# kfjahnke/envutil

Hardware: AMD Instinct MI355X
Metric: Mpix/s reprojected (16K lat/lon->cubemap, b-spline-3) (higher is better)
Workload: dtype f32

## Files before the change

### envutil_amd/csrc/eu_render4.hip

```cpp
#include <cstdio>
#include <cstring>
#include <vector>
#include <algorithm>
#include "eu_packed_dev.h"
#include "eu_launch.h"

#define EU4_TW 16
#define EU4_TH 8
#define EU4_WAVES 4
#ifndef EU4_WAVES0
#define EU4_WAVES0 1
#define EU4_TEXELS 384
#define EU4_OCC0 4
#endif
#define EU4_UNIT_ROWS 4
#define EU4_COL_FLOATS 8
#define EU4_MAX_PLANS 16

__device__ __forceinline__ void eu4_box_reduce(int &mn0, int &mn1, int &mx0, int &mx1)
{
#define EU4_RED(ctrl)                                        \
  "v_min_i32_dpp %0, %0, %0 " ctrl "\n\t"                    \
  "v_min_i32_dpp %1, %1, %1 " ctrl "\n\t"                    \
  "v_max_i32_dpp %2, %2, %2 " ctrl "\n\t"                    \
  "v_max_i32_dpp %3, %3, %3 " ctrl "\n\t"
  asm("s_nop 1\n\t"
      EU4_RED("row_shr:1 row_mask:0xf bank_mask:0xf")
      EU4_RED("row_shr:2 row_mask:0xf bank_mask:0xf")
      EU4_RED("row_shr:4 row_mask:0xf bank_mask:0xf")
      EU4_RED("row_shr:8 row_mask:0xf bank_mask:0xf")
      EU4_RED("row_bcast:15 row_mask:0xa bank_mask:0xf")
      EU4_RED("row_bcast:31 row_mask:0xc bank_mask:0xf")
      "s_nop 0"
      : "+v"(mn0), "+v"(mn1), "+v"(mx0), "+v"(mx1));
#undef EU4_RED
  mn0 = __builtin_amdgcn_readlane(mn0, 63); mn1 = __builtin_amdgcn_readlane(mn1, 63);
  mx0 = __builtin_amdgcn_readlane(mx0, 63); mx1 = __builtin_amdgcn_readlane(mx1, 63);
}

typedef __attribute__((address_space(3))) void *eu4_lds_void;
typedef const __attribute__((address_space(1))) void *eu4_gbl_void;

typedef float eu4_f4 __attribute__((ext_vector_type(4)));

__device__ __forceinline__ void eu4_dma_row(unsigned dst, unsigned voff, const char *sb)
{
  unsigned keep;
  asm volatile("s_mov_b32 %0, m0\n\t"
               "s_mov_b32 m0, %1\n\t"
               "s_nop 0\n\t"
               "global_load_lds_dwordx4 %2, %3\n\t"
               "s_mov_b32 m0, %0"
               : "=&s"(keep) : "s"(dst), "v"(voff), "s"(sb) : "memory");
}

struct eu4_plan {
  const float *atab_g;
  const int *tileplan;
  const float *coltab;
  int tiles16;
  const int *l2_rows;
  int l2_off[9];
  int l2_half;
  unsigned long long l2_magic;
  const int *l1_ent;
  int l1_off[9];
  int l1_ecols;
  unsigned long long l1_magic;
  const int *xtab;
  const int *boxtab;
#ifdef EU5_STAMPS
  unsigned long long *stamps;
#endif
};

#ifdef EU5_STAMPS
#define EU5_STAMP(k) do { asm volatile("" ::: "memory"); st_[k] = __builtin_amdgcn_s_memtime(); asm volatile("" ::: "memory"); } while (0)
#define EU5_STAMP32(k) do { asm volatile("" ::: "memory"); st_[k] = (unsigned)__builtin_amdgcn_s_memtime(); asm volatile("" ::: "memory"); } while (0)
#else
#define EU5_STAMP(k) do { } while (0)
#define EU5_STAMP32(k) do { } while (0)
#endif

template <int NCH, int DEG, int PRJ>
__device__ __forceinline__ void eu4_tile(const eu_render_params &p, const eu4_plan &w, const float *atab,
                                         float *wtile, int tile_y, int x0, int lane)
{
  constexpr int TEX = 4;
  constexpr int order = DEG + 1;
  const eu_src_dev &s = p.src;
  const int lx = lane & 7, ly = lane >> 3;
  const int y = p.row_begin + tile_y * EU4_TH + ly;
  const bool yin = y < p.row_end;
  const int yc = yin ? y : p.row_end - 1;
  const float *rt = p.row + (long long)eu_frame_row(yc, p.band_shift, p.band_count, p.band_index) * EU_ROW_FLOATS;
  const int xa = x0 + 2 * lx, xb = xa + 1;
  const bool va = yin && xa < p.width, vb = yin && xb < p.width;
  const int xac = xa < p.width ? xa : p.width - 1, xbc = xb < p.width ? xb : p.width - 1;

  eu_f2 tx, ty, gy;
  eu_i2 hit, ok = { -1, -1 };
  int ixa, ixb;
  float wxa[order], wxb[order];
  eu_ray2 r;
  {
    const float A0 = rt[0], A1 = rt[1], A2 = rt[2], B0 = rt[3], B1 = rt[4], B2 = rt[5];
    const eu_f2 c0 = { p.col[xac], p.col[xbc] };
    if (p.form == EU_FORM_BCA) {
      const float C0 = rt[6], C1 = rt[7], C2 = rt[8];
      const float *colB = p.col + p.width;
      const eu_f2 c1 = { colB[xac], colB[xbc] };
      r.x = B0 * c0 + C0 * c1 + A0;
      r.y = B1 * c0 + C1 * c1 + A1;
      r.z = B2 * c0 + C2 * c1 + A2;
    } else {
      r.x = B0 * c0 + A0;
      r.y = B1 * c0 + A1;
// ... 114 lines not shown
  if constexpr (EU4_WAVES0 > 1) {
    asm volatile("s_waitcnt vmcnt(0)" ::: "memory");
    __syncthreads();
  }
  if (tile_x >= w.tiles16) return;
  eu4_tile<NCH, DEG, PRJ>(p, w, atab, tile, tile_y, tile_x * EU4_TW, lane);
}

template <int NCH, int DEG, int PRJ>
__device__ __forceinline__ void eu4_direct_tile(const eu_render_params &p, const float *atab, int tile_y, int x0, int lane)
{
  const eu_src_dev &s = p.src;
  const int lx = lane & 7, ly = lane >> 3;
  const int y = p.row_begin + tile_y * EU4_TH + ly;
  const bool yin = y < p.row_end;
  const int yc = yin ? y : p.row_end - 1;
  const float *rt = p.row + (long long)eu_frame_row(yc, p.band_shift, p.band_count, p.band_index) * EU_ROW_FLOATS;
  const int xa = x0 + 2 * lx, xb = xa + 1;
  const bool va = yin && xa < p.width, vb = yin && xb < p.width;
  const int xac = xa < p.width ? xa : p.width - 1, xbc = xb < p.width ? xb : p.width - 1;
  eu_ray2 ry;
  {
    const float A0 = rt[0], A1 = rt[1], A2 = rt[2], B0 = rt[3], B1 = rt[4], B2 = rt[5];
    const eu_f2 c0 = { p.col[xac], p.col[xbc] };
    if (p.form == EU_FORM_BCA) {
      const float C0 = rt[6], C1 = rt[7], C2 = rt[8];
      const float *colB = p.col + p.width;
      const eu_f2 c1 = { colB[xac], colB[xbc] };
      ry.x = B0 * c0 + C0 * c1 + A0;
      ry.y = B1 * c0 + C1 * c1 + A1;
      ry.z = B2 * c0 + C2 * c1 + A2;
    } else {
      ry.x = B0 * c0 + A0;
      ry.y = B1 * c0 + A1;
      ry.z = B2 * c0 + A2;
    }
    if (p.norm_mode == EU_NORM_DIV) {
      eu_f2 sqn = ry.x * ry.x; sqn = sqn + ry.y * ry.y; sqn = sqn + ry.z * ry.z;
      const eu_f2 n = { sqrtf(sqn.x), sqrtf(sqn.y) };
      ry.x = ry.x / n; ry.y = ry.y / n; ry.z = ry.z / n;
    }
  }
  eu_f2 sx, sy;
  eu_i2 hit = eu_coord2<PRJ>(s, ry, sx, sy, atab);
  hit = hit & (eu_i2){ va ? -1 : 0, vb ? -1 : 0 };
  float pxa[NCH], pxb[NCH];
  eu_eval2<NCH, DEG>(s, sx, sy, hit, pxa, pxb);
  float *const orow = p.out + (long long)(yc - p.row_begin) * p.out_stride;
  if (va) eu_put<NCH>(orow, xa, pxa);
  if (vb) eu_put<NCH>(orow, xb, pxb);
}

#include "eu_share_groups.h"
#include "eu_render5.h"

template <int DEG>
__global__ __launch_bounds__(256) void eu_colplan_kernel(const eu_render_params p, float *ct,
                                                         float A0, float A2, float B0, float B2)
{
  __shared__ __attribute__((aligned(16))) float atab[EU_ATAN_TAB_FLOATS];
  if (threadIdx.x < EU_ATAN_TAB_ENTRIES) eu_atan_tab_entry(threadIdx.x, atab + 8 * threadIdx.x);
  __syncthreads();
  constexpr int order = DEG + 1;
  const eu_src_dev &s = p.src;
  const int xa = 2 * (blockIdx.x * 256 + threadIdx.x), xb = xa + 1;
  if (xa >= p.width) return;
  const int xbc = xb < p.width ? xb : p.width - 1;
  const eu_f2 c0 = { p.col[xa], p.col[xbc] };
  const eu_f2 rx = B0 * c0 + A0, rz = B2 * c0 + A2;
  eu_i2 ok = { -1, -1 };
  const eu_f2 q2 = rx * rx + rz * rz;
  const eu_f2 qs = eu_sqrt2_ok(q2, ok);
  const eu_f2 lon = eu_atan2f_2_tab_ok(rx, rz, atab, 0, ok);
  eu_f2 i0 = { (float)((double)lon.x - s.tex_x0), (float)((double)lon.y - s.tex_x0) };
  if (s.cdiv_ok) i0 = eu_div2_const(i0, s.ext_w, s.rcp_ext_w);
  else i0 = i0 / s.ext_w;
  i0 = i0 * s.total_w; i0 = i0 - .5f;
  const eu_f2 sx = i0 - s.win_x_off;
  const eu_f2 gx = eu_gate2_ok(sx, s.gate0, s.lower0, s.upper0, ok);
  eu_f2 fx;
  if constexpr (DEG & 1) fx = (eu_f2){ floorf(gx.x), floorf(gx.y) };
  else fx = (eu_f2){ roundf(gx.x), roundf(gx.y) };
  const eu_f2 tx = gx - fx;
  eu_f2 wx[4];
#pragma unroll
  for (int i = 0; i < 4; i++) wx[i] = (eu_f2){ 0.0f, 0.0f };
  if constexpr (DEG >= 2) eu_weights2<DEG>(s.wm, tx, wx);
  float e[2][EU4_COL_FLOATS];
  e[0][0] = __int_as_float(ok.x ? (int)fx.x : INT_MIN);
  e[1][0] = __int_as_float(ok.y ? (int)fx.y : INT_MIN);
  e[0][1] = tx.x; e[1][1] = tx.y;
#pragma unroll
  for (int i = 0; i < 4; i++) { e[0][2 + i] = i < order ? wx[i].x : 0.0f; e[1][2 + i] = i < order ? wx[i].y : 0.0f; }
  e[0][6] = qs.x; e[1][6] = qs.y;
  e[0][7] = lon.x; e[1][7] = lon.y;
  float *o = ct + (size_t)xa * EU4_COL_FLOATS;
#pragma unroll
  for (int i = 0; i < EU4_COL_FLOATS; i++) o[i] = e[0][i];
  if (xb < p.width) {
#pragma unroll
    for (int i = 0; i < EU4_COL_FLOATS; i++) o[EU4_COL_FLOATS + i] = e[1][i];
  }
}

template <int NCH, int DEG, int PRJ>
__global__ __launch_bounds__(256, 4) void eu_render4d_kernel(const eu_render_params p, const eu4_plan w)
// ... 63 lines not shown
      static const int occ = [] { int n = 0; return hipOccupancyMaxActiveBlocksPerMultiprocessor(&n, eu_render5_kernel<NCH, DEG, PRJ, true>, 64 * EU5_WAVES, 0) == hipSuccess ? n : 0; }();
      per_cu = occ;
    } else {
      static const int occ = [] { int n = 0; return hipOccupancyMaxActiveBlocksPerMultiprocessor(&n, eu_render5_kernel<NCH, DEG, PRJ, false>, 64 * EU5_WAVES, 0) == hipSuccess ? n : 0; }();
      per_cu = occ;
    }
    const int wgs = (cus / 8) * 8 * per_cu;
    if (wgs <= 0) return -1;
    if (fast) eu4_followers_last = eu4_followers_plan;
    eu4_boxtab_last = bt;
    if (bt) hipLaunchKernelGGL((eu_render5_kernel<NCH, DEG, PRJ, true, true>), dim3((unsigned)wgs), dim3(64 * EU5_WAVES), 0, st, p, w);
    else if (fast) hipLaunchKernelGGL((eu_render5_kernel<NCH, DEG, PRJ, true>), dim3((unsigned)wgs), dim3(64 * EU5_WAVES), 0, st, p, w);
    else hipLaunchKernelGGL((eu_render5_kernel<NCH, DEG, PRJ, false>), dim3((unsigned)wgs), dim3(64 * EU5_WAVES), 0, st, p, w);
  } else {
    const int units = (p.tiles_y + EU4_UNIT_ROWS - 1) / EU4_UNIT_ROWS;
    dim3 grid((unsigned)(8 * ((w.tiles16 + EU4_WAVES0 - 1) / EU4_WAVES0)), (unsigned)EU4_UNIT_ROWS, (unsigned)((units + 7) / 8));
    hipLaunchKernelGGL((eu_render4s_kernel<NCH, DEG, PRJ>), grid, dim3(64 * EU4_WAVES0), 0, st, p, w);
  }
  if (hipGetLastError() != hipSuccess) return -1;
  hipLaunchKernelGGL((eu_render4d_kernel<NCH, DEG, PRJ>), dim3(EU4_DIRECT_WGS), dim3(256), 0, st, p, w);
  if (hipGetLastError() != hipSuccess) {
    (void)hipMemsetAsync(p.wl, 0, EU4_WL_ENTRIES * sizeof(int), st);
    return -1;
  }
  return 0;
}

template <int NCH, int DEG>
static int launch4_nd(const eu_render_params &p, const eu4_plan &w, hipStream_t st)
{
  switch (p.src.prj) {
    case EU_SPHERICAL: return launch4_ndp<NCH, DEG, EU_SPHERICAL>(p, w, st);
    case EU_CUBEMAP: return launch4_ndp<NCH, DEG, EU_CUBEMAP>(p, w, st);
    case EU_BIATAN6: return launch4_ndp<NCH, DEG, EU_BIATAN6>(p, w, st);
  }
  return -2;
}

template <int NCH>
static int launch4_n(const eu_render_params &p, const eu4_plan &w, hipStream_t st)
{
  switch (p.src.degree) {
    case 1: return launch4_nd<NCH, 1>(p, w, st);
    case 2: return launch4_nd<NCH, 2>(p, w, st);
    case 3: return launch4_nd<NCH, 3>(p, w, st);
  }
  return -2;
}

static_assert(EU_STAGED_TILE_ROWS == EU4_TH && EU_STAGED_MAX_TILES_Y == 65535 * 8 * EU4_UNIT_ROWS, "eu_select.h: eu_staged_covers");
namespace {
struct plan_cache {
  std::vector<unsigned char> key;
  eu_dev_buf<int> tileplan, l2_rows, l1_ent, xtab, boxtab;
  bool has_boxtab = false;
  long long boxtab_tiles = 0;
  eu_dev_buf<float> coltab;
  float *atab = nullptr;
  int planned_rows = 0;
  int l2_off[9] = {};
  int l1_off[9] = {};
  int l1_ecols = 1;
  long long follower_tiles = 0;
  hipStream_t last_stream = nullptr;
} g4s[EU_MAX_SLOTS];
#define g4 (g4s[eu_current_slot()])

bool ensure_atab()
{
  if (g4.atab) return true;
  std::vector<float> tab(768, 0.0f);
  for (int i = 0; i < EU_ATAN_TAB_ENTRIES; i++) eu_atan_tab_entry(i, tab.data() + 8 * i);
  if (hipMalloc((void **)&g4.atab, tab.size() * sizeof(float)) != hipSuccess) return false;
  return hipMemcpy(g4.atab, tab.data(), tab.size() * sizeof(float), hipMemcpyHostToDevice) == hipSuccess;
}

template <int DEG>
void launch_colplan(const eu_render_params &p, float *ct, const float *k, hipStream_t st)
{
  hipLaunchKernelGGL((eu_colplan_kernel<DEG>), dim3((unsigned)((p.width + 511) / 512)), dim3(256), 0, st, p, ct,
                     k[0], k[1], k[2], k[3]);
}

std::vector<unsigned char> eu4_plan_key(const eu_render_params &p, unsigned long long plan_gen, const eu_switches &sw)
{
  std::vector<unsigned char> key(sizeof(unsigned long long) + sizeof(eu_src_dev) + 11 * sizeof(int));
  unsigned char *q = key.data();
  memcpy(q, &plan_gen, sizeof plan_gen); q += sizeof plan_gen;
  eu_src_dev sd = p.src; sd.base = nullptr;
  memcpy(q, &sd, sizeof sd); q += sizeof sd;
  const int v[11] = { p.width, p.row_begin, p.row_end, p.band_shift, p.band_count, p.band_index, p.form, p.norm_mode, sw.share,
                      sw.boxtab, sw.boxtab_max_kb };
  memcpy(q, v, sizeof v);
  return key;
}

bool upload(eu_dev_buf<int> &buf, const std::vector<int> &v, size_t spare)
{
  if (buf.reserve(v.size() + spare) != hipSuccess) return false;
  return v.empty() || hipMemcpy(buf.p, v.data(), v.size() * sizeof(int), hipMemcpyHostToDevice) == hipSuccess;
}

template <int DEG>
void launch_boxplan(const eu_render_params &p, const float *atab_g, const int *l2_rows, int tiles16, int ntiles, int *tab, hipStream_t st)
{
  hipLaunchKernelGGL((eu5_boxplan_kernel<DEG>), dim3((unsigned)((ntiles + 3) / 4)), dim3(256), 0, st, p, atab_g, l2_rows, tiles16,
                     ntiles, tab);
}

int eu4_build_plans(const eu_render_params &p, int tiles16, const eu_switches &sw, const float *h_row,
                    size_t h_row_floats, hipStream_t st)
{
  std::vector<int> tp((size_t)p.tiles_y, -1);
  std::vector<float> plans;
  const bool can = p.form == EU_FORM_BA && p.norm_mode == EU_NORM_NONE && h_row;
  if (can && sw.colplan) {
    for (int ty = 0; ty < p.tiles_y; ty++) {
      float k[4] = { 0, 0, 0, 0 };
      bool same = true;
      for (int ly = 0; ly < EU4_TH && same; ly++) {
        const int y = std::min(p.row_begin + ty * EU4_TH + ly, p.row_end - 1);
        const size_t fr = (size_t)eu_frame_row(y, p.band_shift, p.band_count, p.band_index) * EU_ROW_FLOATS;
        if (fr + 6 > h_row_floats) { same = false; break; }
        const float c[4] = { h_row[fr + 0], h_row[fr + 2], h_row[fr + 3], h_row[fr + 5] };
        if (ly == 0) memcpy(k, c, sizeof k);
        else same = memcmp(k, c, sizeof k) == 0;
      }
      if (!same) continue;
      int id = -1;
      for (size_t j = 0; j < plans.size() / 4 && id < 0; j++)
        if (memcmp(&plans[4 * j], k, sizeof k) == 0) id = (int)j;
      if (id < 0 && plans.size() / 4 < EU4_MAX_PLANS) {
        id = (int)(plans.size() / 4);
        plans.insert(plans.end(), k, k + 4);
      }
      tp[(size_t)ty] = id;
    }
  }
  const int nplans = (int)(plans.size() / 4);
  if (g4.tileplan.reserve(tp.size()) != hipSuccess) return -1;
  if (g4.coltab.reserve(std::max<size_t>(1, nplans) * (size_t)p.width * EU4_COL_FLOATS) != hipSuccess) return -1;
  if (hipStreamSynchronize(st) != hipSuccess) return -1;
  if (g4.last_stream && g4.last_stream != st && hipStreamSynchronize(g4.last_stream) != hipSuccess) return -1;
  if (hipMemcpy(g4.tileplan.p, tp.data(), tp.size() * sizeof(int), hipMemcpyHostToDevice) != hipSuccess) return -1;
  g4.planned_rows = 0;
  for (int v : tp) g4.planned_rows += v >= 0;
  auto paired = [&](int m) { return 2 * m + 1 < p.tiles_y && tp[(size_t)2 * m] >= 0 && tp[(size_t)2 * m] == tp[(size_t)2 * m + 1]; };
  {
    std::vector<int> rows[8], all;
    for (int r = 0; r < p.tiles_y; r++)
      if (!paired(r >> 1)) rows[(r / EU5_UNIT_ROWS) & 7].push_back(r);
    for (int x = 0; x < 8; x++) { g4.l2_off[x] = (int)all.size(); all.insert(all.end(), rows[x].begin(), rows[x].end()); }
    g4.l2_off[8] = (int)all.size();
    if (!upload(g4.l2_rows, all, 1)) return -1;
  }
  g4.has_boxtab = false; g4.boxtab_tiles = 0;
  if (sw.boxtab && eu_staged_fast_profile(p)) {
    const long long ntiles = (long long)g4.l2_off[8] * tiles16;
    const long long bytes = ntiles * (EU5_BT_RECS * 16);
    if (bytes <= (long long)sw.boxtab_max_kb * 1024) {
      if (g4.boxtab.reserve((size_t)std::max<long long>(1, ntiles) * (EU5_BT_RECS * 4)) != hipSuccess) return -1;
      if (ntiles > 0) {
        switch (p.src.degree) {
          case 1: launch_boxplan<1>(p, g4.atab, g4.l2_rows.p, tiles16, (int)ntiles, g4.boxtab.p, st); break;
          case 2: launch_boxplan<2>(p, g4.atab, g4.l2_rows.p, tiles16, (int)ntiles, g4.boxtab.p, st); break;
          default: launch_boxplan<3>(p, g4.atab, g4.l2_rows.p, tiles16, (int)ntiles, g4.boxtab.p, st); break;
        }
        if (hipGetLastError() != hipSuccess) return -1;
      }
      g4.has_boxtab = true; g4.boxtab_tiles = ntiles;
    }
  }
  for (int j = 0; j < nplans; j++) {
    float *ct = g4.coltab.p + j * (size_t)p.width * EU4_COL_FLOATS;
    switch (p.src.degree) {
      case 1: launch_colplan<1>(p, ct, &plans[4 * j], st); break;
      case 2: launch_colplan<2>(p, ct, &plans[4 * j], st); break;
      default: launch_colplan<3>(p, ct, &plans[4 * j], st); break;
    }
    if (hipGetLastError() != hipSuccess) return -1;
  }
  std::vector<float> h_ct((size_t)nplans * p.width * EU4_COL_FLOATS);
  if (nplans) {
    if (hipStreamSynchronize(st) != hipSuccess) return -1;
    if (hipMemcpy(h_ct.data(), g4.coltab.p, h_ct.size() * sizeof(float), hipMemcpyDeviceToHost) != hipSuccess) return -1;
  }
  std::vector<int> cm, cp;
  for (int m = 0; 2 * m + 1 < p.tiles_y; m++)
    if (paired(m)) { cm.push_back(m); cp.push_back(tp[(size_t)2 * m]); }
  eu_share_input in;
  in.width = p.width; in.tiles16 = tiles16; in.row_begin = p.row_begin; in.row_end = p.row_end;
  in.band_mode = p.band_count > 1;
  in.ncand = (int)cm.size(); in.cand_m = cm.data(); in.cand_plan = cp.data();
  in.h_row = h_row; in.h_row_floats = h_row_floats; in.row_floats = EU_ROW_FLOATS;
  in.coltab = nplans ? h_ct.data() : nullptr; in.col_floats = EU4_COL_FLOATS; in.nplans = nplans;
  in.mode = sw.share; in.unit_drows = EU5_UNIT_ROWS / 2;
  eu_share_result gr;
  eu_share_build(in, gr);
  if (!upload(g4.l1_ent, gr.entries, 2)) return -1;
  if (g4.xtab.reserve(gr.xtab.size()) != hipSuccess) return -1;
  if (hipMemcpy(g4.xtab.p, gr.xtab.data(), gr.xtab.size() * sizeof(int), hipMemcpyHostToDevice) != hipSuccess) return -1;
  for (int x = 0; x < 9; x++) g4.l1_off[x] = gr.off[x];
  g4.l1_ecols = gr.ecols;
  g4.follower_tiles = gr.follower_tiles;
  return 0;
}

void eu4_fill_plan(eu4_plan &w)
{
  w.tileplan = g4.tileplan.p;
  w.coltab = g4.coltab.p;
  w.l2_rows = g4.l2_rows.p;
  for (int x = 0; x < 9; x++) w.l2_off[x] = g4.l2_off[x];
  w.l2_half = (w.tiles16 + 1) / 2;
  w.l2_magic = (1ull << 40) / (unsigned long long)w.l2_half + 1;
  w.l1_ent = g4.l1_ent.p;
  for (int x = 0; x < 9; x++) w.l1_off[x] = g4.l1_off[x];
  w.l1_ecols = g4.l1_ecols;
  w.l1_magic = (1ull << 40) / (unsigned long long)w.l1_ecols + 1;
  w.xtab = g4.xtab.p;
  w.boxtab = g4.has_boxtab ? g4.boxtab.p : nullptr;
}

int launch4(const eu_render_params &p, const eu4_plan &w, hipStream_t st)
{
  switch (p.nch) {
    case 3: return launch4_n<3>(p, w, st);
    case 4: return launch4_n<4>(p, w, st);
  }
  return -2;
}

#ifdef EU5_STAMPS
int launch4_stamped(const eu_render_params &p, eu4_plan &w, hipStream_t st)
{
  static unsigned long long *d_st = nullptr; static size_t st_cap = 0; static int dumps = 0;
  const size_t ntile_st = (size_t)w.tiles16 * p.tiles_y * 8;
  const size_t nst = ntile_st + 8192 * 4;
  if (st_cap < nst) { if (d_st) (void)hipFree(d_st); if (hipMalloc((void **)&d_st, nst * 8) != hipSuccess) return -1; st_cap = nst; }
  (void)hipMemsetAsync(d_st, 0, nst * 8, st);
  w.stamps = d_st;
  const int rc_ = launch4(p, w, st);
  if (rc_ == 0 && dumps < 2 && nst >= 8 * 4096) {
    dumps++;
    std::vector<unsigned long long> h(nst);
    (void)hipStreamSynchronize(st);
    (void)hipMemcpy(h.data(), d_st, nst * 8, hipMemcpyDeviceToHost);
    double acc[32][8] = {}; size_t cnt[32] = {};
    for (size_t t = 0; t < ntile_st / 8; t++) {
      const unsigned long long *q = &h[t * 8];
      if (!q[0] || !q[7]) continue;
      const int cls = (int)(q[1] & 31);
      cnt[cls]++;
      acc[cls][0] += (double)(q[2] - q[0]); acc[cls][1] += (double)(q[3] - q[2]);
      if (q[4]) { acc[cls][2] += (double)(q[4] - q[3]); acc[cls][3] += (double)(q[5] - q[4]); acc[cls][4] += (double)(q[6] - q[5]); }
      acc[cls][5] += (double)(q[7] - q[6]); acc[cls][6] += (double)(q[7] - q[0]);
    }
    {
      double mn = 1e30, mx = 0, sum = 0, l1 = 0, first = 1e30, last = 0; size_t nw = 0;
      for (size_t k = 0; k < 8192; k++) {
        const unsigned long long *q = &h[ntile_st + k * 4];
        if (!q[3]) continue;
        const double d = (double)(q[2] - q[0]);
        mn = std::min(mn, d); mx = std::max(mx, d); sum += d; l1 += (double)(q[1] - q[0]); nw++;
        first = std::min(first, (double)q[0]); last = std::max(last, (double)q[2]);
      }
      if (nw) fprintf(stderr, "eu5 waves: %zu, cycles per wave min %.0f avg %.0f max %.0f, first loop avg %.0f, first start .. last end %.0f\n",
                      nw, mn, sum / nw, mx, l1 / nw, last - first);
// ... 44 lines not shown
```

### envutil_amd/csrc/eu_render5.h

```cpp
#define EU5_WAVES 4
#ifndef EU5_TEXELS
#define EU5_TEXELS 576
#endif
#ifndef EU5_OCC
#define EU5_OCC 4
#endif
#ifndef EU5_UNIT_ROWS
#define EU5_UNIT_ROWS 4
#endif

typedef const __attribute__((address_space(3))) eu4_f4 *eu5_l4ptr;

template <int NCH, int DEG>
__device__ __forceinline__ void eu5_taps(eu_lptr lt, int a, int b, int pitch, const eu_f2 *wx, const eu_f2 *wy,
                                         eu_f2 tx, eu_f2 ty, eu_f2 &rga, eu_f2 &bxa, eu_f2 &rgb, eu_f2 &bxb)
{
  constexpr int order = DEG + 1;
  if constexpr (DEG == 1) {
    const eu_f2 wl0 = 1.0f - tx, wr0 = tx, wl1 = 1.0f - ty, wr1 = ty;
    const eu4_f4 a00 = *(eu5_l4ptr)(lt + a), a01 = *(eu5_l4ptr)(lt + a + 4);
    const eu4_f4 a10 = *(eu5_l4ptr)(lt + a + pitch), a11 = *(eu5_l4ptr)(lt + a + pitch + 4);
    const eu4_f4 b00 = *(eu5_l4ptr)(lt + b), b01 = *(eu5_l4ptr)(lt + b + 4);
    const eu4_f4 b10 = *(eu5_l4ptr)(lt + b + pitch), b11 = *(eu5_l4ptr)(lt + b + pitch + 4);
    {
// ... 943 lines not shown
  if (PRJ != EU_CUBEMAP && wave == 0) {
#pragma unroll
    for (int i = 0; i < 3; i++)
      __builtin_amdgcn_global_load_lds((eu4_gbl_void)(w.atab_g + i * 256 + lane0 * 4),
                                       (eu4_lds_void)(atab + i * 256), 16, 0, 0);
    asm volatile("s_waitcnt vmcnt(0)" ::: "memory");
  }
  __syncthreads();
#ifdef EU5_STAMPS
  const unsigned long long ws0 = __builtin_amdgcn_s_memtime();
  unsigned long long ws1 = ws0;
#endif
  const int xcd = (int)(blockIdx.x & 7);
  const int K = (int)(gridDim.x >> 3) * EU5_WAVES;
  const int t0 = (int)(blockIdx.x >> 3) * EU5_WAVES + wave;
  constexpr bool PAIRS = FAST && PRJ == EU_SPHERICAL;
  if constexpr (PAIRS) {
    const int n1 = (w.l1_off[xcd + 1] - w.l1_off[xcd]) * w.l1_ecols;
    const eu5_cint ents = (eu5_cint)w.l1_ent + EU_SHARE_ENTRY_INTS * w.l1_off[xcd];
    int pos1 = t0;
    auto seek = [&](eu5_cint &e, int &n, int &m, int &plan, int &tcol) -> bool {
      if (pos1 >= n1) return false;
      const int r = (int)(((unsigned long long)(unsigned)pos1 * w.l1_magic) >> 40);
      e = ents + EU_SHARE_ENTRY_INTS * r;
      n = e[0]; m = e[2]; plan = e[3];
      const unsigned h = ((unsigned)m * 0x9E3779B1u) >> 16;
      int c = pos1 - r * w.l1_ecols + (int)((h * (unsigned)w.l1_ecols) >> 16);
      if (c >= w.l1_ecols) c -= w.l1_ecols;
      tcol = e[1] + c;
      pos1 += K;
      return true;
    };
    eu5_cint e_a = ents, e_n = ents;
    int n_a = 0, m_a = 0, col_a = 0, plan_a = 0, n_n = 0, m_n = 0, col_n = 0, plan_n = 0;
    bool have_a = seek(e_a, n_a, m_a, plan_a, col_a);
    eu5_tab16 T;
    if (have_a) eu5_load16(p, w.coltab + (size_t)plan_a * p.width * EU4_COL_FLOATS, 2 * m_a, col_a * EU4_TW, lane0, T);
#pragma unroll 1
    while (have_a) {
      const bool have_n = seek(e_n, n_n, m_n, plan_n, col_n);
      eu5_group16<NCH, DEG>(p, w, atab, tile, T, e_a, n_a, m_a, plan_a, col_a, lane0, have_n, m_n, have_n ? plan_n : 0, col_n);
      e_a = e_n; n_a = n_n; m_a = m_n; plan_a = plan_n; col_a = col_n; have_a = have_n;
    }
  }
#ifdef EU5_STAMPS
  ws1 = __builtin_amdgcn_s_memtime();
#endif
  eu5_iter<EU5_UNIT_ROWS> it;
  it.xcd = xcd; it.tiles16 = w.tiles16;
  it.units = (p.tiles_y + EU5_UNIT_ROWS - 1) / EU5_UNIT_ROWS;
  it.start(t0, K);
  if constexpr (PAIRS) {
    int *const queue = p.wl + EU4_WL_DYN(xcd);
    const int nbatch = (w.l2_off[xcd + 1] - w.l2_off[xcd]) * w.l2_half;
    const eu5_cint rows2 = (eu5_cint)w.l2_rows + w.l2_off[xcd];
    auto take = [&]() -> int {
      int v = 0;
      if (lane0 == 0) v = atomicAdd(queue, 1);
      return v;
    };
    if constexpr (BOXTAB) {
      static_assert(FAST && PRJ == EU_SPHERICAL, "the box table is that of the FAST lat/lon second loop");
      const eu5_crec bt = (eu5_crec)w.boxtab;
      auto decode = [&](int j, int &ty, int &tcol, int &ti) -> bool {
        if (j >= nbatch) return false;
        const int r = (int)(((unsigned long long)(unsigned)j * w.l2_magic) >> 40);
        ty = rows2[r]; tcol = 2 * (j - r * w.l2_half);
        ti = ((w.l2_off[xcd] + r) * w.tiles16 + tcol) * EU5_BT_RECS;
        return true;
      };
      int ty_a = 0, col_a = 0, ti_a = 0, ty_n = 0, col_n = 0, ti_n = 0;
      bool have = decode(__builtin_amdgcn_readfirstlane(take()), ty_a, col_a, ti_a);
      eu5_tab8 Ta, Tb;
      eu5_i4 Ra = { 0, 0, -1, 0 }, Rb = { 0, 0, -1, 0 };
      if (have) { Ra = bt[ti_a]; eu5_load8<FAST>(p, ty_a, col_a * EU4_TW, lane0, Ta); }
      __builtin_amdgcn_s_waitcnt(EU5_WAIT_VM0);
#pragma unroll 1
      while (have) {
        const int jn_lane = take();
        const bool second = col_a + 1 < w.tiles16;
        if (second) Rb = bt[ti_a + EU5_BT_RECS];
        {
          int lane = lane0;
          asm volatile("" : "+v"(lane));
          eu5_tile_bt<NCH, DEG>(p, w, atab, tile, ty_a, col_a * EU4_TW, lane, Ta, Ra, bt + ti_a, second, ty_a,
                                (col_a + 1) * EU4_TW, Tb);
        }
        const bool have_n = decode(__builtin_amdgcn_readfirstlane(jn_lane), ty_n, col_n, ti_n);
        if (have_n) Ra = bt[ti_n];
        if (second) {
          int lane = lane0;
          asm volatile("" : "+v"(lane));
          eu5_tile_bt<NCH, DEG>(p, w, atab, tile, ty_a, (col_a + 1) * EU4_TW, lane, Tb, Rb, bt + ti_a + EU5_BT_RECS, have_n,
                                ty_n, col_n * EU4_TW, Ta);
        } else if (have_n) {
          eu5_load8<FAST>(p, ty_n, col_n * EU4_TW, lane0, Ta);
          __builtin_amdgcn_s_waitcnt(EU5_WAIT_VM0);
        }
        ty_a = ty_n; col_a = col_n; ti_a = ti_n; have = have_n;
      }
    } else {
      auto decode = [&](int j, int &ty, int &tcol) -> bool {
        if (j >= nbatch) return false;
        const int r = (int)(((unsigned long long)(unsigned)j * w.l2_magic) >> 40);
        ty = rows2[r]; tcol = 2 * (j - r * w.l2_half);
        return true;
      };
      int ty_a = 0, col_a = 0, ty_n = 0, col_n = 0;
      bool have = decode(__builtin_amdgcn_readfirstlane(take()), ty_a, col_a);
      eu5_tab8 Ta, Tb;
      if (have) eu5_load8<FAST>(p, ty_a, col_a * EU4_TW, lane0, Ta);
  #pragma unroll 1
      while (have) {
        const int jn_lane = take();
        const bool second = col_a + 1 < w.tiles16;
        {
          int lane = lane0;
          asm volatile("" : "+v"(lane));
          eu5_tile<NCH, DEG, PRJ, false, FAST, true>(p, w, atab, tile, nullptr, ty_a, col_a * EU4_TW, lane, &Ta, second, ty_a,
                                                     (col_a + 1) * EU4_TW, &Tb);
        }
        const bool have_n = decode(__builtin_amdgcn_readfirstlane(jn_lane), ty_n, col_n);
        if (second) {
          int lane = lane0;
          asm volatile("" : "+v"(lane));
          eu5_tile<NCH, DEG, PRJ, false, FAST, true>(p, w, atab, tile, nullptr, ty_a, (col_a + 1) * EU4_TW, lane, &Tb, have_n, ty_n,
                                                     col_n * EU4_TW, &Ta);
        } else if (have_n) eu5_load8<FAST>(p, ty_n, col_n * EU4_TW, lane0, Ta);
        ty_a = ty_n; col_a = col_n; have = have_n;
      }
    }
  } else {
    int plan_n = (it.done() || it.row() >= p.tiles_y) ? -2 : (PRJ == EU_SPHERICAL ? ((eu5_cint)w.tileplan)[it.row()] : -1);
#pragma unroll 1
    while (!it.done()) {
      const int tile_y = it.row(), tcol = it.col(), plan = plan_n;
      it.step();
      plan_n = (it.done() || it.row() >= p.tiles_y) ? -2 : (PRJ == EU_SPHERICAL ? ((eu5_cint)w.tileplan)[it.row()] : -1);
      if (plan == -2) continue;
      int lane = lane0;
      asm volatile("" : "+v"(lane));
      if (plan >= 0)
        eu5_tile<NCH, DEG, PRJ, PRJ == EU_SPHERICAL, FAST>(p, w, atab, tile, w.coltab + (size_t)plan * p.width * EU4_COL_FLOATS,
                                                            tile_y, tcol * EU4_TW, lane);
      else
        eu5_tile<NCH, DEG, PRJ, false, FAST>(p, w, atab, tile, nullptr, tile_y, tcol * EU4_TW, lane);
    }
  }
#ifdef EU5_STAMPS
  if (lane0 == 0 && w.stamps) {
    unsigned long long *o = w.stamps + (size_t)w.tiles16 * p.tiles_y * 8 + ((size_t)blockIdx.x * EU5_WAVES + wave) * 4;
    o[0] = ws0; o[1] = ws1; o[2] = __builtin_amdgcn_s_memtime(); o[3] = 1;
  }
#endif
}
```

### envutil_amd/csrc/eu_select.h

```cpp
#ifndef EU_SELECT_H
#define EU_SELECT_H
#include <algorithm>
#include <climits>
#include <cstdlib>
#include <vector>
#include "eu_device.h"
#include "eu_share_groups.h"
#include "eu_worklist.h"

struct eu_switches {
  int force_general;
  int hybrid;
  int r4;
  int colmajor;
  int rej;
  int colplan;
  int share;
  int direct;
  int iir_stream;
  int boxtab;
  int boxtab_max_kb;
  int views_max_kb;
};

#define EU_BOXTAB_MAX_KB 65536
#define EU_VIEWS_MAX_KB 65536

inline eu_switches eu_read_switches()
{
  auto first = [](const char *name) { const char *e = getenv(name); return e ? e[0] : '\0'; };
  eu_switches s;
  s.force_general = first("EU_HIP_KERNEL") == '1';
  const char hy = first("EU_HIP_HYBRID");
  s.hybrid = hy == '0' ? 0 : hy == '2' ? 2 : 1;
  const char *r4 = getenv("EU_HIP_R4");
  s.r4 = r4 ? atoi(r4) : -1;
  const char *cm = getenv("EU_HIP_COLMAJOR");
  s.colmajor = cm && cm[0] ? atoi(cm) : -1;
  const char rj = first("EU_HIP_REJ");
  s.rej = rj == '1' ? 1 : rj == '2' ? 2 : 0;
  s.colplan = first("EU_HIP_COLPLAN") != '0';
  const char sh = first("EU_HIP_SHARE");
  s.share = sh == '0' ? 0 : sh == 'm' ? EU_SHARE_MIRRORS : sh == 'f' ? EU_SHARE_FACES : EU_SHARE_FACES | EU_SHARE_MIRRORS;
  s.direct = first("EU_HIP_DIRECT") == '1';
  const char *iir = getenv("EU_HIP_IIR_STREAM");
  s.iir_stream = iir ? atoi(iir) : 7;
  s.boxtab = first("EU_HIP_BOXTAB") != '0';
  const char *bm = getenv("EU_HIP_BOXTAB_MAX_KB");
  s.boxtab_max_kb = bm && bm[0] ? std::max(0, std::min(atoi(bm), 16 * 1024 * 1024)) : EU_BOXTAB_MAX_KB;
  const char *vm = getenv("EU_HIP_VIEWS_MAX_KB");
  s.views_max_kb = vm && vm[0] ? std::max(0, std::min(atoi(vm), 16 * 1024 * 1024)) : EU_VIEWS_MAX_KB;
  return s;
}

inline bool eu_cube_source(int prj) { return prj == EU_CUBEMAP || prj == EU_BIATAN6; }

inline bool eu_packed_covers_source(const eu_src_dev &s, int nch, int nch_out)
{
  if (s.has_lcp || nch_out != nch) return false;
  if (s.prj != EU_SPHERICAL && !eu_cube_source(s.prj)) return false;
  if (s.degree < 1 || s.degree > 3 || s.es0 != nch) return false;
  return nch >= 1 && nch <= 4;
}
inline bool eu_packed_covers(const eu_render_params &p)
{
  if (p.stage != 0 || p.form >= EU_FORM_FISH) return false;
  return eu_packed_covers_source(p.src, p.nch, p.nch_out);
}

#define EU_STAGED_TILE_ROWS 8
#define EU_STAGED_TILE_COLS 16
#define EU_STAGED_MAX_TILES_Y (65535 * 8 * 4)
inline unsigned long long eu_staged_tiles(int width, int row_begin, int row_end)
{
  const long long tx = ((long long)width + EU_STAGED_TILE_COLS - 1) / EU_STAGED_TILE_COLS;
  const long long ty = ((long long)row_end - row_begin + EU_STAGED_TILE_ROWS - 1) / EU_STAGED_TILE_ROWS;
  return tx > 0 && ty > 0 ? (unsigned long long)tx * (unsigned long long)ty : 0ull;
}
inline bool eu_staged_covers(const eu_render_params &p)
{
  if (!eu_packed_covers(p) || p.twine) return false;
  if (p.norm_mode != EU_NORM_NONE && p.norm_mode != EU_NORM_DIV) return false;
  if (p.nch != 3 && p.nch != 4) return false;
  if (p.src.es1 * 4 >= (1ll << 31)) return false;
  if ((p.row_end - p.row_begin + EU_STAGED_TILE_ROWS - 1) / EU_STAGED_TILE_ROWS > EU_STAGED_MAX_TILES_Y) return false;
  return eu_staged_tiles(p.width, p.row_begin, p.row_end) <= EU4_WL_MAX_TILES;
}

inline bool eu_plain_ba(const eu_render_params &p)
{
  return p.form == EU_FORM_BA && p.norm_mode == EU_NORM_NONE && p.band_count <= 1 && p.src.brighten == 1.0f &&
         p.src.always_hit;
}

inline bool eu_staged_default(const eu_render_params &p)
{
  return p.src.prj == EU_SPHERICAL && p.src.degree >= 2 && !p.twine && eu_plain_ba(p);
}

inline bool eu_staged_fast_profile(const eu_render_params &p)
{
  auto mag_ok = [](double v) { const double a = v < 0 ? -v : v; return a == 0.0 || (a >= 0x1p-20 && a <= 0x1p20); };
  return eu_plain_ba(p) && mag_ok(p.src.tex_x0) && mag_ok(p.src.tex_y0) && p.src.ext_w >= 0x1p-20f &&
         p.src.ext_w <= 0x1p20f && p.src.ext_h >= 0x1p-20f && p.src.ext_h <= 0x1p20f && p.tab_finite;
// ... 80 lines not shown
```

Measured before the change: 111,900.

## Replace per-XCD row lists with configurable block walk for tile scheduling

The row-major second-loop worklist, which bucketed rows by unit index per XCD and decoded jobs with a magic divide, is replaced by a block-structured walk. The output is split into blocks of H rows by C column pairs, with blocks distributed across XCDs and jobs decoded by shifts and masks, so consecutive jobs touch nearby source data for better L2 reuse. The first-loop share unit size can also be chosen adaptively. The default shape (4 rows, full width) is close to the old one, and padded slots inside a block are now skipped as empty jobs, which adds some wasted queue entries.

```diff
diff --git a/envutil_amd/csrc/eu_render4.hip b/envutil_amd/csrc/eu_render4.hip
--- a/envutil_amd/csrc/eu_render4.hip
+++ b/envutil_amd/csrc/eu_render4.hip
@@ -59,10 +59,9 @@
   const int *tileplan;
   const float *coltab;
   int tiles16;
-  const int *l2_rows;
-  int l2_off[9];
-  int l2_half;
-  unsigned long long l2_magic;
+  const int *l2_blk;
+  int l2_boff[9];
+  int l2_shape;
   const int *l1_ent;
   int l1_off[9];
   int l1_ecols;
@@ -283,6 +282,7 @@
 }
 
 #include "eu_share_groups.h"
+#include "eu_walk.h"
 #include "eu_render5.h"
 
 template <int DEG>
@@ -452,13 +452,16 @@
 namespace {
 struct plan_cache {
   std::vector<unsigned char> key;
-  eu_dev_buf<int> tileplan, l2_rows, l1_ent, xtab, boxtab;
+  eu_dev_buf<int> tileplan, l2_rows, l2_blk, l1_ent, xtab, boxtab;
   bool has_boxtab = false;
   long long boxtab_tiles = 0;
   eu_dev_buf<float> coltab;
   float *atab = nullptr;
   int planned_rows = 0;
-  int l2_off[9] = {};
+  int l2_nrows = 0;
+  int l2_boff[9] = {};
+  int l2_hs = 0, l2_cs = 0, l2_order = 0;
+  int l1_unit = 2;
   int l1_off[9] = {};
   int l1_ecols = 1;
   long long follower_tiles = 0;
@@ -484,13 +487,13 @@
 
 std::vector<unsigned char> eu4_plan_key(const eu_render_params &p, unsigned long long plan_gen, const eu_switches &sw)
 {
-  std::vector<unsigned char> key(sizeof(unsigned long long) + sizeof(eu_src_dev) + 11 * sizeof(int));
+  std::vector<unsigned char> key(sizeof(unsigned long long) + sizeof(eu_src_dev) + 15 * sizeof(int));
   unsigned char *q = key.data();
   memcpy(q, &plan_gen, sizeof plan_gen); q += sizeof plan_gen;
   eu_src_dev sd = p.src; sd.base = nullptr;
   memcpy(q, &sd, sizeof sd); q += sizeof sd;
-  const int v[11] = { p.width, p.row_begin, p.row_end, p.band_shift, p.band_count, p.band_index, p.form, p.norm_mode, sw.share,
-                      sw.boxtab, sw.boxtab_max_kb };
+  const int v[15] = { p.width, p.row_begin, p.row_end, p.band_shift, p.band_count, p.band_index, p.form, p.norm_mode, sw.share,
+                      sw.boxtab, sw.boxtab_max_kb, sw.walk.l1_drows, sw.walk.l2_rows, sw.walk.l2_pairs, sw.walk.l2_order };
   memcpy(q, v, sizeof v);
   return key;
 }
@@ -547,16 +550,20 @@
   for (int v : tp) g4.planned_rows += v >= 0;
   auto paired = [&](int m) { return 2 * m + 1 < p.tiles_y && tp[(size_t)2 * m] >= 0 && tp[(size_t)2 * m] == tp[(size_t)2 * m + 1]; };
   {
-    std::vector<int> rows[8], all;
+    std::vector<int> all;
     for (int r = 0; r < p.tiles_y; r++)
-      if (!paired(r >> 1)) rows[(r / EU5_UNIT_ROWS) & 7].push_back(r);
-    for (int x = 0; x < 8; x++) { g4.l2_off[x] = (int)all.size(); all.insert(all.end(), rows[x].begin(), rows[x].end()); }
-    g4.l2_off[8] = (int)all.size();
+      if (!paired(r >> 1)) all.push_back(r);
+    eu_walk_l2 wk;
+    eu_walk_build_l2(all.data(), (int)all.size(), (tiles16 + 1) / 2, sw.walk, wk);
+    g4.l2_nrows = (int)all.size();
+    for (int x = 0; x < 9; x++) g4.l2_boff[x] = wk.off[x];
+    g4.l2_hs = wk.hs; g4.l2_cs = wk.cs; g4.l2_order = wk.order;
+    if (!upload(g4.l2_blk, wk.blocks, EU_WALK_BLOCK_INTS)) return -1;
     if (!upload(g4.l2_rows, all, 1)) return -1;
   }
   g4.has_boxtab = false; g4.boxtab_tiles = 0;
   if (sw.boxtab && eu_staged_fast_profile(p)) {
-    const long long ntiles = (long long)g4.l2_off[8] * tiles16;
+    const long long ntiles = (long long)g4.l2_nrows * tiles16;
     const long long bytes = ntiles * (EU5_BT_RECS * 16);
     if (bytes <= (long long)sw.boxtab_max_kb * 1024) {
       if (g4.boxtab.reserve((size_t)std::max<long long>(1, ntiles) * (EU5_BT_RECS * 4)) != hipSuccess) return -1;
@@ -594,9 +601,15 @@
   in.ncand = (int)cm.size(); in.cand_m = cm.data(); in.cand_plan = cp.data();
   in.h_row = h_row; in.h_row_floats = h_row_floats; in.row_floats = EU_ROW_FLOATS;
   in.coltab = nplans ? h_ct.data() : nullptr; in.col_floats = EU4_COL_FLOATS; in.nplans = nplans;
-  in.mode = sw.share; in.unit_drows = EU5_UNIT_ROWS / 2;
+  in.mode = sw.share; in.unit_drows = 2;
   eu_share_result gr;
   eu_share_build(in, gr);
+  {
+    std::vector<int> leaders;
+    for (size_t e = 0; e + EU_SHARE_ENTRY_INTS <= gr.entries.size(); e += EU_SHARE_ENTRY_INTS) leaders.push_back(gr.entries[e + 2]);
+    g4.l1_unit = eu_walk_l1_unit(leaders.data(), (int)leaders.size(), sw.walk.l1_drows);
+    if (g4.l1_unit != in.unit_drows) { in.unit_drows = g4.l1_unit; eu_share_build(in, gr); }
+  }
   if (!upload(g4.l1_ent, gr.entries, 2)) return -1;
   if (g4.xtab.reserve(gr.xtab.size()) != hipSuccess) return -1;
   if (hipMemcpy(g4.xtab.p, gr.xtab.data(), gr.xtab.size() * sizeof(int), hipMemcpyHostToDevice) != hipSuccess) return -1;
@@ -610,10 +623,9 @@
 {
   w.tileplan = g4.tileplan.p;
   w.coltab = g4.coltab.p;
-  w.l2_rows = g4.l2_rows.p;
-  for (int x = 0; x < 9; x++) w.l2_off[x] = g4.l2_off[x];
-  w.l2_half = (w.tiles16 + 1) / 2;
-  w.l2_magic = (1ull << 40) / (unsigned long long)w.l2_half + 1;
+  w.l2_blk = g4.l2_blk.p;
+  for (int x = 0; x < 9; x++) w.l2_boff[x] = g4.l2_boff[x];
+  w.l2_shape = g4.l2_hs | g4.l2_cs << 8 | g4.l2_order << 16;
   w.l1_ent = g4.l1_ent.p;
   for (int x = 0; x < 9; x++) w.l1_off[x] = g4.l1_off[x];
   w.l1_ecols = g4.l1_ecols;
diff --git a/envutil_amd/csrc/eu_render5.h b/envutil_amd/csrc/eu_render5.h
--- a/envutil_amd/csrc/eu_render5.h
+++ b/envutil_amd/csrc/eu_render5.h
@@ -1019,81 +1019,81 @@
   it.start(t0, K);
   if constexpr (PAIRS) {
     int *const queue = p.wl + EU4_WL_DYN(xcd);
-    const int nbatch = (w.l2_off[xcd + 1] - w.l2_off[xcd]) * w.l2_half;
-    const eu5_cint rows2 = (eu5_cint)w.l2_rows + w.l2_off[xcd];
+    const int nbatch = (w.l2_boff[xcd + 1] - w.l2_boff[xcd]) << ((w.l2_shape & 31) + ((w.l2_shape >> 8) & 31));
+    const eu5_crec blks = (eu5_crec)w.l2_blk + w.l2_boff[xcd];
     auto take = [&]() -> int {
       int v = 0;
       if (lane0 == 0) v = atomicAdd(queue, 1);
       return v;
     };
+    auto decode = [&](int j, int &ty, int &tcol, int &ti) -> bool {
+      ty = -1;
+      if (j >= nbatch) return false;
+      int shape = w.l2_shape;
+      asm volatile("" : "+s"(shape));
+      const int hs = shape & 31, cs = (shape >> 8) & 31;
+      int i, lr, lc;
+      const eu5_i4 B = blks[eu_walk_block_of(j, hs, cs, i)];
+      const bool is = eu_walk_in_block(i, hs, cs, shape >> 16, B.w, lr, lc);
+      ty = is ? B.y + lr : -1; tcol = 2 * (B.z + lc);
+      ti = ((B.x + lr) * w.tiles16 + tcol) * EU5_BT_RECS;
+      return true;
+    };
     if constexpr (BOXTAB) {
       static_assert(FAST && PRJ == EU_SPHERICAL, "the box table is that of the FAST lat/lon second loop");
       const eu5_crec bt = (eu5_crec)w.boxtab;
-      auto decode = [&](int j, int &ty, int &tcol, int &ti) -> bool {
-        if (j >= nbatch) return false;
-        const int r = (int)(((unsigned long long)(unsigned)j * w.l2_magic) >> 40);
-        ty = rows2[r]; tcol = 2 * (j - r * w.l2_half);
-        ti = ((w.l2_off[xcd] + r) * w.tiles16 + tcol) * EU5_BT_RECS;
-        return true;
-      };
       int ty_a = 0, col_a = 0, ti_a = 0, ty_n = 0, col_n = 0, ti_n = 0;
       bool have = decode(__builtin_amdgcn_readfirstlane(take()), ty_a, col_a, ti_a);
       eu5_tab8 Ta, Tb;
       eu5_i4 Ra = { 0, 0, -1, 0 }, Rb = { 0, 0, -1, 0 };
-      if (have) { Ra = bt[ti_a]; eu5_load8<FAST>(p, ty_a, col_a * EU4_TW, lane0, Ta); }
+      if ((ty_a >= 0)) { Ra = bt[ti_a]; eu5_load8<FAST>(p, ty_a, col_a * EU4_TW, lane0, Ta); }
       __builtin_amdgcn_s_waitcnt(EU5_WAIT_VM0);
 #pragma unroll 1
       while (have) {
         const int jn_lane = take();
-        const bool second = col_a + 1 < w.tiles16;
+        const bool second = (ty_a >= 0) && col_a + 1 < w.tiles16;
         if (second) Rb = bt[ti_a + EU5_BT_RECS];
-        {
+        if ((ty_a >= 0)) {
           int lane = lane0;
           asm volatile("" : "+v"(lane));
           eu5_tile_bt<NCH, DEG>(p, w, atab, tile, ty_a, col_a * EU4_TW, lane, Ta, Ra, bt + ti_a, second, ty_a,
                                 (col_a + 1) * EU4_TW, Tb);
         }
         const bool have_n = decode(__builtin_amdgcn_readfirstlane(jn_lane), ty_n, col_n, ti_n);
-        if (have_n) Ra = bt[ti_n];
+        if ((ty_n >= 0)) Ra = bt[ti_n];
         if (second) {
           int lane = lane0;
           asm volatile("" : "+v"(lane));
-          eu5_tile_bt<NCH, DEG>(p, w, atab, tile, ty_a, (col_a + 1) * EU4_TW, lane, Tb, Rb, bt + ti_a + EU5_BT_RECS, have_n,
+          eu5_tile_bt<NCH, DEG>(p, w, atab, tile, ty_a, (col_a + 1) * EU4_TW, lane, Tb, Rb, bt + ti_a + EU5_BT_RECS, (ty_n >= 0),
                                 ty_n, col_n * EU4_TW, Ta);
-        } else if (have_n) {
+        } else if ((ty_n >= 0)) {
           eu5_load8<FAST>(p, ty_n, col_n * EU4_TW, lane0, Ta);
           __builtin_amdgcn_s_waitcnt(EU5_WAIT_VM0);
         }
         ty_a = ty_n; col_a = col_n; ti_a = ti_n; have = have_n;
       }
     } else {
-      auto decode = [&](int j, int &ty, int &tcol) -> bool {
-        if (j >= nbatch) return false;
-        const int r = (int)(((unsigned long long)(unsigned)j * w.l2_magic) >> 40);
-        ty = rows2[r]; tcol = 2 * (j - r * w.l2_half);
-        return true;
-      };
-      int ty_a = 0, col_a = 0, ty_n = 0, col_n = 0;
-      bool have = decode(__builtin_amdgcn_readfirstlane(take()), ty_a, col_a);
+      int ty_a = 0, col_a = 0, ty_n = 0, col_n = 0, ti_ = 0;
+      bool have = decode(__builtin_amdgcn_readfirstlane(take()), ty_a, col_a, ti_);
       eu5_tab8 Ta, Tb;
-      if (have) eu5_load8<FAST>(p, ty_a, col_a * EU4_TW, lane0, Ta);
+      if ((ty_a >= 0)) eu5_load8<FAST>(p, ty_a, col_a * EU4_TW, lane0, Ta);
   #pragma unroll 1
       while (have) {
         const int jn_lane = take();
-        const bool second = col_a + 1 < w.tiles16;
-        {
+        const bool second = (ty_a >= 0) && col_a + 1 < w.tiles16;
+        if ((ty_a >= 0)) {
           int lane = lane0;
           asm volatile("" : "+v"(lane));
           eu5_tile<NCH, DEG, PRJ, false, FAST, true>(p, w, atab, tile, nullptr, ty_a, col_a * EU4_TW, lane, &Ta, second, ty_a,
                                                      (col_a + 1) * EU4_TW, &Tb);
         }
-        const bool have_n = decode(__builtin_amdgcn_readfirstlane(jn_lane), ty_n, col_n);
+        const bool have_n = decode(__builtin_amdgcn_readfirstlane(jn_lane), ty_n, col_n, ti_);
         if (second) {
           int lane = lane0;
           asm volatile("" : "+v"(lane));
-          eu5_tile<NCH, DEG, PRJ, false, FAST, true>(p, w, atab, tile, nullptr, ty_a, (col_a + 1) * EU4_TW, lane, &Tb, have_n, ty_n,
+          eu5_tile<NCH, DEG, PRJ, false, FAST, true>(p, w, atab, tile, nullptr, ty_a, (col_a + 1) * EU4_TW, lane, &Tb, (ty_n >= 0), ty_n,
                                                      col_n * EU4_TW, &Ta);
-        } else if (have_n) eu5_load8<FAST>(p, ty_n, col_n * EU4_TW, lane0, Ta);
+        } else if ((ty_n >= 0)) eu5_load8<FAST>(p, ty_n, col_n * EU4_TW, lane0, Ta);
         ty_a = ty_n; col_a = col_n; have = have_n;
       }
     }
diff --git a/envutil_amd/csrc/eu_select.h b/envutil_amd/csrc/eu_select.h
--- a/envutil_amd/csrc/eu_select.h
+++ b/envutil_amd/csrc/eu_select.h
@@ -3,9 +3,11 @@
 #include <algorithm>
 #include <climits>
 #include <cstdlib>
+#include <cstring>
 #include <vector>
 #include "eu_device.h"
 #include "eu_share_groups.h"
+#include "eu_walk.h"
 #include "eu_worklist.h"
 
 struct eu_switches {
@@ -21,6 +23,7 @@
   int boxtab;
   int boxtab_max_kb;
   int views_max_kb;
+  eu_walk_shape walk;
 };
 
 #define EU_BOXTAB_MAX_KB 65536
@@ -50,6 +53,19 @@
   s.boxtab_max_kb = bm && bm[0] ? std::max(0, std::min(atoi(bm), 16 * 1024 * 1024)) : EU_BOXTAB_MAX_KB;
   const char *vm = getenv("EU_HIP_VIEWS_MAX_KB");
   s.views_max_kb = vm && vm[0] ? std::max(0, std::min(atoi(vm), 16 * 1024 * 1024)) : EU_VIEWS_MAX_KB;
+  s.walk = eu_walk_shape EU_WALK_DEFAULT_INIT;
+  if (const char *wk = getenv("EU_HIP_WALK")) {
+    if (wk[0] == 'p') s.walk = eu_walk_shape EU_WALK_PARENT_INIT;
+    else {
+      const char *f[4] = { wk, nullptr, nullptr, nullptr };
+      for (int k = 1; k < 4 && f[k - 1]; k++) { const char *c = strchr(f[k - 1], ','); f[k] = c ? c + 1 : nullptr; }
+      auto given = [](const char *q) { return q && q[0] && q[0] != ','; };
+      if (given(f[0])) { const int u = atoi(f[0]); if (u == 0 || u == 2 || u == 4 || u == 8) s.walk.l1_drows = u; }
+      if (given(f[1])) { const int h = atoi(f[1]); if (eu_walk_pow2(h) && h <= EU_WALK_MAX_H) s.walk.l2_rows = h; }
+      if (given(f[2])) { const int c = atoi(f[2]); if (c == 0 || (eu_walk_pow2(c) && c <= EU_WALK_MAX_C)) s.walk.l2_pairs = c; }
+      if (given(f[3])) s.walk.l2_order = f[3][0] == 'c';
+    }
+  }
   return s;
 }
 
diff --git a/envutil_amd/csrc/eu_walk.h b/envutil_amd/csrc/eu_walk.h
--- /dev/null
+++ b/envutil_amd/csrc/eu_walk.h
@@ -0,0 +1,99 @@
+#ifndef EU_WALK_H
+#define EU_WALK_H
+#include <vector>
+
+#if defined(__HIPCC__) || defined(__CUDACC__)
+#define EU_WALK_HD __host__ __device__ __forceinline__
+#else
+#define EU_WALK_HD inline
+#endif
+
+struct eu_walk_shape {
+  int l1_drows;
+  int l2_rows;
+  int l2_pairs;
+  int l2_order;
+};
+#define EU_WALK_MAX_H 4096
+#define EU_WALK_MAX_C 4096
+#define EU_WALK_PARENT_INIT { 2, 4, 0, 0 }
+#define EU_WALK_DEFAULT_INIT { 2, 4, 0, 0 }
+
+struct eu_walk_block {
+  int slot0;
+  int ty0;
+  int cp0;
+  int ext;
+};
+#define EU_WALK_BLOCK_INTS 4
+
+inline int eu_walk_log2_ceil(int v) { int s = 0; while ((1 << s) < v && s < 30) s++; return s; }
+inline bool eu_walk_pow2(int v) { return v > 0 && (v & (v - 1)) == 0; }
+
+EU_WALK_HD bool eu_walk_in_block(int i, int hs, int cs, int order, int ext, int &lr, int &lc)
+{
+  if (order) { lr = i & ((1 << hs) - 1); lc = i >> hs; }
+  else { lc = i & ((1 << cs) - 1); lr = i >> cs; }
+  return lr < (ext & 0xffff) && lc < (int)((unsigned)ext >> 16);
+}
+EU_WALK_HD int eu_walk_block_of(int j, int hs, int cs, int &i)
+{
+  i = j & ((1 << (hs + cs)) - 1);
+  return j >> (hs + cs);
+}
+
+struct eu_walk_l2 {
+  std::vector<int> blocks;
+  int off[9];
+  int hs, cs, order;
+};
+
+inline void eu_walk_build_l2(const int *rows, int nrows, int half, const eu_walk_shape &sh, eu_walk_l2 &out)
+{
+  int H = eu_walk_pow2(sh.l2_rows) && sh.l2_rows <= EU_WALK_MAX_H ? sh.l2_rows : 4;
+  int hs = eu_walk_log2_ceil(H);
+  const int full = eu_walk_log2_ceil(half > 1 ? half : 1);
+  int cs = eu_walk_pow2(sh.l2_pairs) && sh.l2_pairs <= EU_WALK_MAX_C ? eu_walk_log2_ceil(sh.l2_pairs) : full;
+  if (cs > full) cs = full;
+  const int tall = eu_walk_log2_ceil(nrows > 0 ? rows[nrows - 1] + 1 : 1);
+  if (hs > tall) hs = tall;
+  const int bcols = half > 0 ? (half + (1 << cs) - 1) >> cs : 0;
+  while (hs > 0 && ((long long)nrows * bcols << (hs + cs)) > (1ll << 30)) hs--;
+  H = 1 << hs;
+  std::vector<int> lists[8];
+  for (int a = 0; a < nrows;) {
+    int b = a + 1;
+    while (b < nrows && rows[b] == rows[b - 1] + 1 && (rows[b] & (H - 1)) != 0) b++;
+    const int R = rows[a] >> hs;
+    for (int q = 0; q < bcols; q++) {
+      const int cp0 = q << cs;
+      const int ncp = half - cp0 < (1 << cs) ? half - cp0 : (1 << cs);
+      std::vector<int> &l = lists[(R + q) & 7];
+      l.push_back(a); l.push_back(rows[a]); l.push_back(cp0); l.push_back((b - a) | (ncp << 16));
+    }
+    a = b;
+  }
+  out.blocks.clear();
+  for (int x = 0; x < 8; x++) {
+    out.off[x] = (int)(out.blocks.size() / EU_WALK_BLOCK_INTS);
+    out.blocks.insert(out.blocks.end(), lists[x].begin(), lists[x].end());
+  }
+  out.off[8] = (int)(out.blocks.size() / EU_WALK_BLOCK_INTS);
+  out.hs = hs; out.cs = cs; out.order = sh.l2_order ? 1 : 0;
+}
+
+inline int eu_walk_l1_unit(const int *leader_m, int n, int forced)
+{
+  if (forced == 2 || forced == 4 || forced == 8) return forced;
+  int base[8] = {};
+  for (int k = 0; k < n; k++) base[(leader_m[k] / 2) & 7]++;
+  for (int u = 8; u > 2; u >>= 1) {
+    int cnt[8] = {};
+    for (int k = 0; k < n; k++) cnt[(leader_m[k] / u) & 7]++;
+    bool ok = true;
+    for (int x = 0; x < 8; x++) ok = ok && cnt[x] >= base[x];
+    if (ok) return u;
+  }
+  return 2;
+}
+#endif
```

New measurement: 112,100 (median of 3 runs). No clear change (+0.2%).
